# mmbajo/PROBA-V

Measured on AMD Instinct MI355X. Metric: LR-patches/sec fwd+bwd (WDSR-B r12 t9, 16x16, bs128), higher is better.
Workload: dtype f32 (products as 3 scaled-fp16-piece MFMA products, f32 accumulate)

## Files before the change

### proba-v_amd/csrc/kernels_cw4.hip

```cpp
#include "kernels_x6.h"
#include "x6_device.h"
#include <cstdlib>
#include <algorithm>

namespace probav {
#ifdef CW4_DIAG
namespace diag {
#endif

struct Cw4Args {
    ConvGeom g;
    int Wp, Wt, nsplit, SR, nstrips, nslot;
    unsigned mTo, mNvr, mTi, mNslot;
};

namespace {
__device__ __forceinline__ int qdiv(int v, int d, unsigned m) { return (int)__umulhi((unsigned)v, m) + (d == 1 ? v : 0); }
unsigned qmagic(int d) { return d <= 1 ? 0u : (unsigned)((0x100000000ull + (unsigned)d - 1) / (unsigned)d); }
typedef float f32x4u __attribute__((ext_vector_type(4), aligned(4)));
typedef unsigned u32x4b __attribute__((ext_vector_type(4)));
constexpr int CW4_PSE = 151;
constexpr int CW4_PS = 16 * CW4_PSE;
constexpr int CW4_ROW = 8 * CW4_PS;
constexpr unsigned CW4_OOB = 0x40000000u;
}

#ifdef CW4_STAMP
__device__ unsigned long long g_cw4_stamps[1024 * 8];
#endif

#define CW4_SBAR() __builtin_amdgcn_sched_barrier(0)
#ifdef CW4_STAMP
#define CW4_ST(k) do { unsigned long long t_; asm volatile("s_memtime %0\n\ts_waitcnt lgkmcnt(0)" : "=s"(t_) :: "memory"); st_acc[k] += t_ - st_prev; st_prev = t_; } while (0)
#ifdef CW4_STAMP_ROUNDS
#define CW4_STR(k) CW4_ST(k)
#else
#define CW4_STR(k) do { } while (0)
#endif
#else
#define CW4_STR(k) do { } while (0)
#define CW4_ST(k) do { } while (0)
#endif

template <int CIN, int COUT, int TP, bool RELU, bool SKIP, bool BIAS>
__global__ __launch_bounds__(256, 1) void conv3_w4_kernel(Cw4Args a, const float* __restrict__ x, const uint4* __restrict__ wfrag, const float* __restrict__ bias,
                                                         const float* __restrict__ skip, float* __restrict__ y, Amax am)
{
    extern __shared__ __attribute__((aligned(16))) unsigned char lds[];
    constexpr int NST = CIN == 25 ? 5 : 6, KB = 9 * NST, G = 3 * KB;
    constexpr int NW1R = CIN == 25 ? 12 : 8;
    constexpr int NCH = CIN == 25 ? 3 : 4;
    constexpr int PS = CW4_PS, ROW = CW4_ROW;
    constexpr int PD = 2;
    constexpr int TO = TP - 2;
    const ConvGeom& g = a.g;
    const int tid = threadIdx.x, lane = tid & 63, half = lane >> 5, col = lane & 31;
    const int wave = __builtin_amdgcn_readfirstlane(tid >> 6);
    const int per = a.nstrips * a.nsplit;
    const int n = blockIdx.x / per, srem = blockIdx.x - n * per;
    const int strip = srem / a.nsplit, sp = srem - strip * a.nsplit;
    const int ws0 = sp * a.Wt, hb = strip * a.SR;
    const int SRr = g.Ho - hb < a.SR ? g.Ho - hb : a.SR;
    const int nvr = a.Wt * g.To, NV = SRr * nvr, NTL = (NV + 31) >> 5, nround = (NTL + 3) >> 2;
    const int NS = a.nslot;
    float omax = 0.f;
#ifdef CW4_STAMP
    unsigned long long st_t0 = __builtin_amdgcn_s_memtime(), st_r0 = __builtin_amdgcn_s_memrealtime();
    unsigned long long st_prev = st_t0, st_acc[8] = {0, 0, 0, 0, 0, 0, 0, 0};
#endif

    const int lw0 = a.nsplit == 1 ? g.pw : 0, Wl = a.nsplit == 1 ? g.Wi : a.Wt + 2;
    const int nvs = Wl * g.Ti, items = nvs * NCH;
    const int ea = h3_exp(am.x[n]);
    const float sa = pow2i(ea);
    int s_srcb[2], s_offb[2];
    float s_sc[2];
    int s3_o[3], s3_offb = 0;
    float s3_sc[3] = {0.f, 0.f, 0.f};
    {
        auto locate = [&](int lv, int& lw, int& t, int& iwc, int& colok) {
            const int lwr = qdiv(lv, g.Ti, a.mTi);
            t = lv - lwr * g.Ti; lw = lw0 + lwr;
            const int iw = ws0 + lw - g.pw;
            colok = (iw >= 0 ? 1 : 0) & (iw < g.Wi ? 1 : 0);
            iwc = iw < 0 ? 0 : (iw < g.Wi ? iw : g.Wi - 1);
        };
#pragma unroll
        for (int k = 0; k < 2; ++k) {
            const int it = tid + 256 * k;
            const int ic = it < items ? it : items - 1;
            const int lv = CIN == 25 ? (int)(((unsigned)ic * 43691u) >> 17) : ic >> 2;
            const int cc = ic - lv * NCH;
            int lw, t, iwc, colok;
            locate(lv, lw, t, iwc, colok);
            s_srcb[k] = ((iwc * g.Ti + t) * CIN + 8 * cc) * 4;
            s_offb[k] = (lw * TO + t) * 16 + cc * PS;
            s_sc[k] = colok ? sa : 0.f;
        }
        if constexpr (CIN == 25) {
            const int lv = tid < nvs ? tid : nvs - 1;
            int lw, t, iwc, colok;
            locate(lv, lw, t, iwc, colok);
            const int base = ((iwc * g.Ti + t) * CIN + 24) * 4;
            s3_offb = (lw * TO + t) * 16 + 3 * PS;
            const int ok3[3] = {colok && t - 1 >= 0, colok, colok && t + 1 < g.Ti};
#pragma unroll
            for (int j = 0; j < 3; ++j) { s3_o[j] = base + (ok3[j] ? (j - 1) * CIN * 4 : 0); s3_sc[j] = ok3[j] ? sa : 0.f; }
        }
    }
    const long xsample = (long)g.Hi * g.Wi * g.Ti * CIN;
    const __amdgpu_buffer_rsrc_t xrs = __builtin_amdgcn_make_buffer_rsrc(const_cast<float*>(x + (long)n * xsample), 0, (unsigned)xsample * 4u, 0x00020000);
    const int xrowb = g.Wi * g.Ti * CIN * 4;
    struct Staged { u32x4b v[2][2]; unsigned g3[3]; };
    auto row_of = [&](int q, int& rowoff, float& rokf) {
        const int ih = hb - g.ph + q;
        const bool rok = ih >= 0 && ih < g.Hi;
        rowoff = (rok ? ih : 0) * xrowb;
        rokf = rok ? 1.f : 0.f;
    };
    auto stage_load_items = [&](int rowoff, Staged& sv) {
#pragma unroll
        for (int k = 0; k < 2; ++k) {
            sv.v[k][0] = __builtin_amdgcn_raw_buffer_load_b128(xrs, s_srcb[k], rowoff, 0);
            sv.v[k][1] = __builtin_amdgcn_raw_buffer_load_b128(xrs, s_srcb[k] + 16, rowoff, 0);
        }
    };
    auto stage_load_g3 = [&](int rowoff, Staged& sv) {
#ifdef CW4_ABL_NOG3
        sv.g3[0] = sv.g3[1] = sv.g3[2] = 0u; return;
#endif
        if constexpr (CIN == 25) {
#pragma unroll
            for (int j = 0; j < 3; ++j) sv.g3[j] = __builtin_amdgcn_raw_buffer_load_b32(xrs, s3_o[j], rowoff, 0);
        }
    };
    auto slot_of = [&](int q) -> int { return (q - qdiv(q, NS, a.mNslot) * NS) * ROW; };
    struct Cut { float sc[2], sg[3]; f32x2 t[4]; unsigned h0[4], h1[4]; float u[3]; };
    constexpr int ROW_MOPS = CIN == 25 ? 52 : 41;
    auto stage_mop = [&](int m, int slot, float rokf, Staged& sv, Cut& c, bool reload, int rel) {
        if (m < 5) {
            if (m < 2) c.sc[m] = s_sc[m] * rokf;
            else if (CIN == 25) c.sg[m - 2] = s3_sc[m - 2] * rokf;
            return;
        }
        m -= 5;
        if (m < 36) {
            const int k = m / 18, i = m % 18;
            if (i < 16) {
                const int p = i >> 2, op = i & 3;
                if (op == 0) {
                    const u32x4b q = sv.v[k][p >> 1];
                    const f32x2 v = {__uint_as_float(q[2 * (p & 1)]), __uint_as_float(q[2 * (p & 1) + 1])};
                    c.t[p] = v * (f32x2){c.sc[k], c.sc[k]};
                    if (p == 3 && reload) {
                        sv.v[k][0] = __builtin_amdgcn_raw_buffer_load_b128(xrs, s_srcb[k], rel, 0);
                        sv.v[k][1] = __builtin_amdgcn_raw_buffer_load_b128(xrs, s_srcb[k] + 16, rel, 0);
                    }
                } else if (op == 1) {
                    c.h0[p] = __builtin_bit_cast(unsigned, __builtin_convertvector(c.t[p], f16x2));
                } else if (op == 2) {
                    asm("v_fma_mixlo_f16 %0, %1, -1.0, %2 op_sel:[0,0,0] op_sel_hi:[1,0,0]" : "=v"(c.h1[p]) : "v"(c.h0[p]), "v"(c.t[p][0]));
                } else {
                    asm("v_fma_mixhi_f16 %0, %1, -1.0, %2 op_sel:[1,0,0] op_sel_hi:[1,0,0]" : "+v"(c.h1[p]) : "v"(c.h0[p]), "v"(c.t[p][1]));
                }
            } else {
#ifdef CW4_ABL_NOWRITE
                asm volatile("" :: "v"(c.h0[0]), "v"(c.h0[1]), "v"(c.h0[2]), "v"(c.h0[3]), "v"(c.h1[0]), "v"(c.h1[1]), "v"(c.h1[2]), "v"(c.h1[3]));
                return;
#endif
                unsigned char* ent = lds + slot + s_offb[k];
                if (i == 16) *reinterpret_cast<uint4*>(ent) = make_uint4(c.h0[0], c.h0[1], c.h0[2], c.h0[3]);
                else *reinterpret_cast<uint4*>(ent + 4 * PS) = make_uint4(c.h1[0], c.h1[1], c.h1[2], c.h1[3]);
            }
            return;
        }
        if constexpr (CIN == 25) {
            m -= 36;
            if (m < 3) { c.u[m] = __uint_as_float(sv.g3[m]) * c.sg[m]; if (m == 2 && reload) stage_load_g3(rel, sv); }
            else if (m == 3) c.h0[0] = __builtin_bit_cast(unsigned, __builtin_convertvector((f32x2){c.u[0], c.u[1]}, f16x2));
            else if (m == 4) c.h0[1] = __builtin_bit_cast(unsigned, __builtin_convertvector((f32x2){c.u[2], 0.f}, f16x2));
            else if (m == 5) asm("v_fma_mixlo_f16 %0, %1, -1.0, %2 op_sel:[0,0,0] op_sel_hi:[1,0,0]" : "=v"(c.h1[0]) : "v"(c.h0[0]), "v"(c.u[0]));
            else if (m == 6) asm("v_fma_mixhi_f16 %0, %1, -1.0, %2 op_sel:[1,0,0] op_sel_hi:[1,0,0]" : "+v"(c.h1[0]) : "v"(c.h0[0]), "v"(c.u[1]));
            else if (m == 7) c.h1[1] = 0u;
            else if (m == 8) asm("v_fma_mixlo_f16 %0, %1, -1.0, %2 op_sel:[0,0,0] op_sel_hi:[1,0,0]" : "+v"(c.h1[1]) : "v"(c.h0[1]), "v"(c.u[2]));
            else if (m == 9) *reinterpret_cast<uint2*>(lds + slot + s3_offb) = make_uint2(c.h0[0], c.h0[1]);
            else *reinterpret_cast<uint2*>(lds + slot + s3_offb + 4 * PS) = make_uint2(c.h1[0], c.h1[1]);
        }
    };
    auto need = [&](int r) -> int {
        const int vlast = (r + 1) * 128 - 1 < NV - 1 ? (r + 1) * 128 - 1 : NV - 1;
        return qdiv(vlast, nvr, a.mNvr) + 2;
    };

    CW4_ST(3);
    int hiq = nround > 0 ? need(0) : -1;
    Staged p0[4];
    int p0_slot[4];
    float p0_rok[4];
#pragma unroll
    for (int q = 0; q < 4; ++q) {
        int rowoff;
        row_of(q <= hiq ? q : 0, rowoff, p0_rok[q]);
        p0_slot[q] = slot_of(q <= hiq ? q : 0);
        stage_load_items(rowoff, p0[q]);
        stage_load_g3(rowoff, p0[q]);
    }
    constexpr int NQ = ((KB - NW1R) * 64 + 255) / 256;
    u32x4b w1q[NQ];
    const u32x4b* wfrag4 = reinterpret_cast<const u32x4b*>(wfrag);
    const int Z0c = a.Wp * (TP - 2);
    constexpr int NF = KB + NW1R, NF4 = (NF + 3) / 4;
    u32x4b xq[NF4];
#pragma unroll
    for (int i = 0; i < NF4; ++i) {
        int f = 4 * i + wave;
        f = f < NF ? f : NF - 1;
        xq[i] = wfrag4[(f < KB ? 2 * f : 2 * (f - KB) + 1) * 64 + lane];
    }
    const int tab = NS * ROW + (KB - NW1R) * 1024;
    const int tc = tid < g.Cout ? tid : 0;
    const unsigned tew = am.w[tc];
    const float tbv = (bias ? bias : reinterpret_cast<const float*>(am.w))[tc];
#pragma unroll
    for (int i = 0; i < NQ; ++i) {
        int e = tid + 256 * i;
        e = e < (KB - NW1R) * 64 ? e : (KB - NW1R) * 64 - 1;
        w1q[i] = wfrag4[(2 * (NW1R + (e >> 6)) + 1) * 64 + (e & 63)];
    }
    CW4_ST(4);
    if (tid < 32) {
        const int e = -(ea + h3_exp_w(tew));
        reinterpret_cast<int*>(lds + tab)[tid] = e;
        reinterpret_cast<float*>(lds + tab + 128)[tid] = (BIAS && bias && tid < g.Cout) ? ldexpf(tbv, -e) : 0.f;
    }
#pragma unroll
    for (int i = 0; i < NF4; ++i) {
        int f = 4 * i + wave;
        f = f < NF ? f : NF - 1;
        *reinterpret_cast<u32x4b*>(lds + f * 1024 + lane * 16) = xq[i];
    }
    asm volatile("s_waitcnt lgkmcnt(0)\n\ts_barrier" ::: "memory");
    f16x8 w0[KB], w1r[NW1R > 0 ? NW1R : 1];
#pragma unroll
    for (int K = 0; K < KB; ++K) { Frag f; f.u = *reinterpret_cast<const uint4*>(lds + K * 1024 + lane * 16); w0[K] = f.h; }
#pragma unroll
    for (int K = 0; K < NW1R; ++K) { Frag f; f.u = *reinterpret_cast<const uint4*>(lds + (KB + K) * 1024 + lane * 16); w1r[K] = f.h; }
#pragma unroll
    for (int K = 0; K < KB; ++K) asm volatile("" : "+a"(w0[K]));
#pragma unroll
    for (int K = 0; K < NW1R; ++K) asm volatile("" : "+a"(w1r[K]));
    asm volatile("s_waitcnt lgkmcnt(0)\n\ts_barrier" ::: "memory");
    if (a.nsplit == 1) {
        uint4* z = reinterpret_cast<uint4*>(lds);
        for (int i = tid; i < NS * ROW / 16; i += 256) z[i] = make_uint4(0u, 0u, 0u, 0u);
    } else {
        const int nzone = CW4_PSE - Z0c, nplanes = NS * 8;
        for (int i = tid; i < nzone * nplanes; i += 256) {
            const int pl = i / nzone, e = i - pl * nzone;
            *reinterpret_cast<uint4*>(lds + pl * PS + (Z0c + e) * 16) = make_uint4(0u, 0u, 0u, 0u);
        }
        if constexpr (CIN == 25) {
            for (int i = tid; i < Z0c * NS * 2; i += 256) {
                const int pl = i / Z0c, e = i - pl * Z0c;
                *reinterpret_cast<uint4*>(lds + (pl >> 1) * ROW + (3 + 4 * (pl & 1)) * PS + e * 16) = make_uint4(0u, 0u, 0u, 0u);
            }
        }
    }
    asm volatile("s_waitcnt lgkmcnt(0)\n\ts_barrier" ::: "memory");
    CW4_ST(5);
#pragma unroll
    for (int q = 0; q < 4; ++q) {
        Cut c;
#pragma unroll
        for (int m = 0; m < ROW_MOPS; ++m) stage_mop(m, p0_slot[q], p0_rok[q], p0[q], c, false, 0);
    }
    CW4_ST(6);
    const int w1a = NS * ROW + lane * 16;
#pragma unroll
    for (int i = 0; i < NQ; ++i) {
        int e = tid + 256 * i;
        e = e < (KB - NW1R) * 64 ? e : (KB - NW1R) * 64 - 1;
        *reinterpret_cast<u32x4b*>(lds + NS * ROW + e * 16) = w1q[i];
    }
    int eun[16];
    f32x16 bias16;
#pragma unroll
    for (int jj = 0; jj < 4; ++jj) {
        const int4 e4 = *reinterpret_cast<const int4*>(lds + tab + (8 * jj + 4 * half) * 4);
        const float4 b4 = *reinterpret_cast<const float4*>(lds + tab + 128 + (8 * jj + 4 * half) * 4);
        eun[4 * jj] = e4.x; eun[4 * jj + 1] = e4.y; eun[4 * jj + 2] = e4.z; eun[4 * jj + 3] = e4.w;
        bias16[4 * jj] = b4.x; bias16[4 * jj + 1] = b4.y; bias16[4 * jj + 2] = b4.z; bias16[4 * jj + 3] = b4.w;
    }
    const float lo = g.relu ? 0.f : -__builtin_inff();
    (void)lo;
    if (BIAS) asm volatile("" : "+a"(bias16));
    CW4_ST(7);
    asm volatile("s_waitcnt lgkmcnt(0)\n\ts_barrier" ::: "memory");

    const long out_base = ((long)n * g.Ho + hb) * g.Wo * g.To;
    const unsigned ybytes = (unsigned)(SRr * g.Wo * g.To * g.Cout) * 4u;
    const __amdgpu_buffer_rsrc_t yrs = __builtin_amdgcn_make_buffer_rsrc(y + out_base * g.Cout, 0, ybytes, 0x00020000);
    const __amdgpu_buffer_rsrc_t srs = __builtin_amdgcn_make_buffer_rsrc(const_cast<float*>(skip ? skip + out_base * g.Cout : y), 0, skip ? ybytes : 0u, 0x00020000);
    unsigned cofs[4];
#pragma unroll
    for (int jj = 0; jj < 4; ++jj) cofs[jj] = 8 * jj + 4 * half < COUT ? 4u * (8 * jj + 4 * half) : CW4_OOB;

    int offH[5];
    {
        const int pA[5] = {0, 2, 1, 0, 2}, pB[5] = {1, 0, 2, 1, 3};
#pragma unroll
        for (int st = 0; st < 5; ++st) offH[st] = (half ? pB[st] : pA[st]) * PS;
    }
    const int Z0 = a.Wp * TO;
    struct TileTmp { int vi, hrel, rem, w, t, x, e0, s0, s1, s2, b0, b1, b2, dlo, dhi; unsigned yo; };
    constexpr int TILE_STEPS = 14;
    auto tile_step = [&](int step, int tile, TileTmp& q, int (&bs)[9], unsigned (&eo)[4]) {
#define CW4_PIN(v) asm volatile("" : "+v"(v))
        if (step == 0) { const int v = tile * 32 + col; q.vi = v < NV ? v : NV - 1; q.yo = v < NV ? 0u : CW4_OOB; CW4_PIN(q.vi); CW4_PIN(q.yo); }
        if (step == 1) { q.hrel = (int)__umulhi((unsigned)q.vi, a.mNvr); q.rem = q.vi - q.hrel * nvr; CW4_PIN(q.hrel); CW4_PIN(q.rem); }
        if (step == 2) { q.w = (int)__umulhi((unsigned)q.rem, a.mTo); q.t = q.rem - q.w * g.To; CW4_PIN(q.w); CW4_PIN(q.t); }
        if (step == 3) { q.x = q.w * TO + q.t; q.s0 = q.hrel - (int)__umulhi((unsigned)q.hrel, a.mNslot) * NS; CW4_PIN(q.x); CW4_PIN(q.s0); }
        if (step == 4) { q.s1 = q.s0 + 1 < NS ? q.s0 + 1 : q.s0 + 1 - NS; q.e0 = q.x * 16 + (CIN == 32 ? half * PS : 0); CW4_PIN(q.s1); CW4_PIN(q.e0); }
        if (step == 5) { q.s2 = q.s1 + 1 < NS ? q.s1 + 1 : q.s1 + 1 - NS; CW4_PIN(q.s2); }
        if (step == 6) { q.b0 = q.s0 * ROW + q.e0; q.b1 = q.s1 * ROW + q.e0; q.b2 = q.s2 * ROW + q.e0; bs[1] = q.b0; bs[4] = q.b1; bs[7] = q.b2; CW4_PIN(bs[1]); CW4_PIN(bs[4]); CW4_PIN(bs[7]); }
        if (step == 7) { const int z = ((q.x - 1 - Z0) & 15) + Z0 - q.x; q.dlo = q.t == 0 ? z * 16 : -16; CW4_PIN(q.dlo); }
        if (step == 8) { const int z = ((q.x + 1 - Z0) & 15) + Z0 - q.x; q.dhi = q.t == TO - 1 ? z * 16 : 16; CW4_PIN(q.dhi); }
        if (step == 9) { bs[0] = q.b0 + q.dlo; bs[3] = q.b1 + q.dlo; bs[6] = q.b2 + q.dlo; CW4_PIN(bs[0]); CW4_PIN(bs[3]); CW4_PIN(bs[6]); }
        if (step == 10) { bs[2] = q.b0 + q.dhi; bs[5] = q.b1 + q.dhi; bs[8] = q.b2 + q.dhi; CW4_PIN(bs[2]); CW4_PIN(bs[5]); CW4_PIN(bs[8]); }
        if (step == 11) { q.yo += (unsigned)(((q.hrel * g.Wo + ws0 + q.w) * g.To + q.t) * COUT) * 4u; CW4_PIN(q.yo); }
        if (step == 12) { eo[0] = q.yo + cofs[0]; eo[1] = q.yo + cofs[1]; CW4_PIN(eo[0]); CW4_PIN(eo[1]); }
        if (step == 13) { eo[2] = q.yo + cofs[2]; eo[3] = q.yo + cofs[3]; CW4_PIN(eo[2]); CW4_PIN(eo[3]); }
#undef CW4_PIN
    };
    int adr5[5] = {0, 0, 0, 0, 0};
    auto read_A = [&](const int (&bs)[9], int K, Frag (&af)[2]) {
        const int gg = K / NST, st = K % NST, dh = gg / 3, dw = gg % 3;
        if constexpr (CIN == 25) {
            if (dw == 0) {
                const int bm = bs[3 * dh], bz = bs[3 * dh + 1], bp = bs[3 * dh + 2];
                const int b = st == 0 ? bm : st == 1 ? (half ? bz : bm) : st == 2 ? bz : st == 3 ? bp : (half ? bz : bp);
                adr5[st] = b + offH[st];
            }
            const unsigned char* p = lds + adr5[st];
            af[0].u = *reinterpret_cast<const uint4*>(p + dw * TO * 16);
            af[1].u = *reinterpret_cast<const uint4*>(p + dw * TO * 16 + 4 * PS);
        } else {
            const int d = st >> 1, kb = st & 1;
            const unsigned char* p = lds + bs[3 * dh + d];
            af[0].u = *reinterpret_cast<const uint4*>(p + dw * TO * 16 + 2 * kb * PS);
            af[1].u = *reinterpret_cast<const uint4*>(p + dw * TO * 16 + 2 * kb * PS + 4 * PS);
        }
    };
    auto read_W1 = [&](int K, Frag& wf) {
        if (K >= NW1R) wf.u = *reinterpret_cast<const uint4*>(lds + w1a + (K - NW1R) * 1024);
    };

    CW4_ST(2);
    f32x16 accA, accB;
#pragma unroll
    for (int i = 0; i < 16; ++i) { accA[i] = 0.f; accB[i] = 0.f; }
#ifdef CW4_ABL_2ACC
    f32x16 acc2;
    for (int i = 0; i < 16; ++i) acc2[i] = 0.f;
#endif
    f32x4u skq[4];
#pragma unroll
    for (int jj = 0; jj < 4; ++jj) skq[jj] = (f32x4u){0.f, 0.f, 0.f, 0.f};
    int bs[9];
    unsigned eo[4], eo_prev[4] = {CW4_OOB, CW4_OOB, CW4_OOB, CW4_OOB};
    {
        TileTmp q;
#pragma unroll
        for (int st = 0; st < TILE_STEPS; ++st) tile_step(st, wave, q, bs, eo);
    }
    Frag A[PD + 1][2], W1[PD + 1];
#pragma unroll
    for (int K = 0; K < PD; ++K) { read_A(bs, K, A[K]); read_W1(K, W1[K]); }

    Staged sv[2];
    auto round = [&](int r, f32x16& acc, f32x16& pacc) __attribute__((always_inline)) {
        const int hi_next = r + 1 < nround ? need(r + 1) : hiq;
        const int hi_nn = r + 2 < nround ? need(r + 2) : hi_next;
        const int q0 = hiq + 1, q1 = hi_next - hiq >= 2 ? hiq + 2 : hiq + 1;
        const int n0 = hi_next + 1, n1 = hi_nn - hi_next >= 2 ? hi_next + 2 : hi_next + 1;
        int rowoff[2], slot[2];
        float rokf[2], rokn;
        int dummy;
        row_of(q0, dummy, rokf[0]); row_of(q1, dummy, rokf[1]);
        row_of(n0, rowoff[0], rokn); row_of(n1, rowoff[1], rokn);
        slot[0] = slot_of(q0); slot[1] = slot_of(q1);
        Cut cut;
        TileTmp tq;
        int nbs[9];
        unsigned neo[4];
        float m2 = 0.f;
#pragma unroll
        for (int K = 0; K < KB; ++K) {
#pragma unroll
            for (int j = 0; j < 3; ++j) {
                const int gp = 3 * K + j;
                const int sl = K % (PD + 1);
                {
                    f16x8 wa;
                    if (j == 1) { if (K < NW1R) wa = w1r[K < NW1R ? K : 0]; else wa = W1[sl].h; }
                    else wa = w0[K];
                    const f16x8 xb = (j == 0) ? A[sl][1].h : A[sl][0].h;
                    if (gp == 0) {
                        if (BIAS) acc = __builtin_amdgcn_mfma_f32_32x32x16_f16(wa, xb, bias16, 0, 0, 0);
                        else {
                            f32x16 zero;
#pragma unroll
                            for (int i = 0; i < 16; ++i) zero[i] = 0.f;
                            acc = __builtin_amdgcn_mfma_f32_32x32x16_f16(wa, xb, zero, 0, 0, 0);
                        }
                    } else acc = __builtin_amdgcn_mfma_f32_32x32x16_f16(wa, xb, acc, 0, 0, 0);
                }
                CW4_SBAR();
#ifndef CW4_ABL_NOREAD
                if (j == 0) {
                    const int KN = K + PD, sn = KN % (PD + 1);
#ifndef CW4_ABL_W1LATE
                    read_W1(KN < KB ? KN : KN - KB, W1[sn]);
#endif
                    if (KN < KB) read_A(bs, KN, A[sn]); else read_A(nbs, KN - KB, A[sn]);
                }
#ifdef CW4_ABL_W1LATE
                if (j == 1) {
                    const int KN = K + PD, sn = KN % (PD + 1);
                    read_W1(KN < KB ? KN : KN - KB, W1[sn]);
                }
#endif
#endif
                if (K >= 1 && K <= 10 && j == 1) tile_step(K - 1, 4 * (r + 1) + wave, tq, nbs, neo);
                if (K >= 12 && K <= 15 && j == 1) tile_step(K - 2, 4 * (r + 1) + wave, tq, nbs, neo);
                if (K == 11 && j == 1) { CW4_STR(3); asm volatile("s_barrier" ::: "memory"); CW4_STR(4); }
#ifndef CW4_ABL_NOEPI
                if (K < 16 && j == 2) {
                    const int e = K, jj = e >> 2, i = e & 3;
                    float v = ldexpf(pacc[e], eun[e]);
                    if (RELU) v = fmaxf(v, lo);
                    const float o = SKIP ? v + skq[jj][i] : v;
                    skq[jj][i] = o;
                    if ((e & 1) == 0) m2 = o; else asm volatile("v_max3_f32 %0, %0, |%1|, |%2|" : "+v"(omax) : "v"(m2), "v"(o));
                }
                if (j == 1 && (K == 4 || K == 8 || K == 12 || K == 16)) {
                    const int jj = K / 4 - 1;
                    const u32x4b o = {__float_as_uint(skq[jj][0]), __float_as_uint(skq[jj][1]), __float_as_uint(skq[jj][2]), __float_as_uint(skq[jj][3])};
                    if (COUT == 32 || jj < 3) __builtin_amdgcn_raw_buffer_store_b128(o, yrs, eo_prev[jj], 0, 0);
                    else __builtin_amdgcn_raw_buffer_store_b32(o[0], yrs, eo_prev[jj], 0, 0);
                    if (K == 16) omax = r == 0 ? 0.f : omax;
                }
                if (SKIP && (K == 17 || K == 18) && j > 0) {
                    const int jj = 2 * (K - 17) + j - 1;
                    if (COUT == 32 || jj < 3) {
                        const u32x4b q = __builtin_amdgcn_raw_buffer_load_b128(srs, eo[jj], 0, 0);
                        skq[jj] = (f32x4u){__uint_as_float(q[0]), __uint_as_float(q[1]), __uint_as_float(q[2]), __uint_as_float(q[3])};
                    } else {
                        const unsigned q = __builtin_amdgcn_raw_buffer_load_b32(srs, eo[jj], 0, 0);
                        skq[jj] = (f32x4u){__uint_as_float(q), 0.f, 0.f, 0.f};
                    }
                }
#endif
#ifndef CW4_ABL_NOSTAGE
                {
                    constexpr int NKS = (2 * ROW_MOPS + 5) / 6, KS0 = KB - PD - NKS;
                    if (K >= KS0 && K < KS0 + NKS && j > 0) {
                        const int m0 = (K - KS0) * 6 + 3 * (j - 1);
#pragma unroll
                        for (int m = m0; m < m0 + 3; ++m)
                            if (m < 2 * ROW_MOPS) {
#ifdef CW4_ABL_NOCUT
                                if (m == 0) asm volatile("" :: "v"(sv[0].v[0][0]), "v"(sv[0].v[1][1]), "v"(sv[1].v[0][0]), "v"(sv[1].v[1][1]));
                                continue;
#endif
                                stage_mop(m % ROW_MOPS, slot[m / ROW_MOPS], rokf[m / ROW_MOPS], sv[m / ROW_MOPS], cut, true, rowoff[m / ROW_MOPS]);
                            }
                    }
                }
#endif
                CW4_SBAR();
            }
        }
        CW4_STR(5);
#pragma unroll
        for (int d = 0; d < 9; ++d) bs[d] = nbs[d];
#pragma unroll
        for (int jj = 0; jj < 4; ++jj) { eo_prev[jj] = eo[jj]; eo[jj] = neo[jj]; }
        hiq = hi_next;
    };
    {
        const int hi1 = 1 < nround ? need(1) : hiq;
        const int n0 = hiq + 1, n1 = hi1 - hiq >= 2 ? hiq + 2 : hiq + 1;
        int ro;
        float rk;
        row_of(n0, ro, rk); stage_load_items(ro, sv[0]); stage_load_g3(ro, sv[0]);
        row_of(n1, ro, rk); stage_load_items(ro, sv[1]); stage_load_g3(ro, sv[1]);
    }
#pragma unroll 1
    for (int r = 0; r < nround; r += 2) {
        round(r, accA, accB);
        round(r + 1, accB, accA);
    }
    {
#pragma unroll
        for (int e = 0; e < 16; ++e) {
            const int jj = e >> 2, i = e & 3;
            float v = ldexpf(accB[e], eun[e]);
            if (RELU) v = fmaxf(v, lo);
            const float o = SKIP ? v + skq[jj][i] : v;
            skq[jj][i] = o;
            omax = fmaxf(omax, fabsf(o));
        }
        if (nround == 0) omax = 0.f;
#pragma unroll
        for (int jj = 0; jj < 4; ++jj) {
            const u32x4b o = {__float_as_uint(skq[jj][0]), __float_as_uint(skq[jj][1]), __float_as_uint(skq[jj][2]), __float_as_uint(skq[jj][3])};
            if (COUT == 32 || jj < 3) __builtin_amdgcn_raw_buffer_store_b128(o, yrs, eo_prev[jj], 0, 0);
            else __builtin_amdgcn_raw_buffer_store_b32(o[0], yrs, eo_prev[jj], 0, 0);
        }
    }
#ifdef CW4_ABL_2ACC
    for (int i = 0; i < 16; ++i) omax += acc2[i];
#endif
    if (am.y) amax_commit(omax, am.y + n);
#ifdef CW4_STAMP
    if (lane == 0 && blockIdx.x < 256) {
        unsigned long long* o = g_cw4_stamps + (blockIdx.x * 4 + wave) * 8;
        o[0] = __builtin_amdgcn_s_memtime() - st_t0; o[1] = __builtin_amdgcn_s_memrealtime() - st_r0;
        for (int k = 2; k < 8; ++k) o[k] = st_acc[k];
    }
#endif
}

static bool cw4_plan(const ConvGeom& g, Cw4Args& p, size_t& lds_bytes, int& grid)
{
    if (g.kh != 3 || g.kw != 3 || g.kt != 3 || g.reflect_hw || g.reflect_t) return false;
    if (!((g.Cin == 25 && g.Cout == 32) || (g.Cin == 32 && (g.Cout == 25 || g.Cout == 32)))) return false;
    if (g.ph != 1 || g.pw != 1 || g.pt != 1) return false;
    if (g.Ho != g.Hi || g.Wo != g.Wi || g.To != g.Ti) return false;
    if (g.To != 9 && g.To != 7) return false;
    if (g.Ho < 3) return false;
    const int Tp = g.To + 2;
    for (int ns = 1; ns <= 4; ++ns) {
        if (g.Wo % ns) continue;
        const int wt = g.Wo / ns, nvr = wt * g.To;
        const int wp = wt + 2;
        const int nvs = (ns == 1 ? g.Wi : wt + 2) * g.Ti, items = nvs * (g.Cin == 25 ? 3 : 4);
        if (items > 512 || nvs > 256 || nvr < 64 || wp * g.To + 16 + 2 * g.To > CW4_PSE) continue;
        int nstrips = (256 + g.N * ns - 1) / (g.N * ns);
        if (nstrips < 1) nstrips = 1;
        if (nstrips > g.Ho / 4) nstrips = g.Ho / 4 > 0 ? g.Ho / 4 : 1;
        const int SR = (g.Ho + nstrips - 1) / nstrips;
        nstrips = (g.Ho + SR - 1) / SR;
        const int NV = SR * nvr, nround = ((NV + 31) / 32 + 3) / 4;
        auto needf = [&](int r) { const int vl = std::min(NV - 1, (r + 1) * 128 - 1); return vl / nvr + 2; };
        int nslot = needf(0) + 1;
        for (int r = 0; r + 1 < nround; ++r) nslot = std::max(nslot, needf(r + 1) - (r * 128) / nvr + 1);
        const int kb = g.Cin == 25 ? 45 : 54, nw1r = g.Cin == 25 ? 12 : 8;
        const size_t need = (size_t)nslot * CW4_ROW + (size_t)(kb - nw1r) * 1024 + 256;
        if (need > 163840) continue;
        p.g = g; p.Wp = wp; p.Wt = wt; p.nsplit = ns; p.SR = SR; p.nstrips = nstrips; p.nslot = nslot;
        p.mTo = qmagic(g.To); p.mNvr = qmagic(nvr); p.mTi = qmagic(g.Ti); p.mNslot = qmagic(nslot);
        lds_bytes = need; grid = g.N * nstrips * ns;
        return true;
    }
    return false;
}

bool cw4_conv_supported(const ConvGeom& g, const float* gate)
{
    Cw4Args p;
    size_t lds_bytes;
    int grid;
    return gate == nullptr && cw4_plan(g, p, lds_bytes, grid);
}

int cw4_conv_forward(const ConvGeom& g, const float* x, const float* wfrag, const float* bias, const float* skip, float* y, const Amax& am, hipStream_t s)
{
    Cw4Args p;
    size_t lds_bytes;
    int grid;
    if (!cw4_plan(g, p, lds_bytes, grid)) { set_error("cw4_conv_forward: unsupported geometry", hipSuccess); return PROBAV_EINVAL; }
    if (!am.x || !am.w) { set_error("cw4_conv_forward: H3 arithmetic needs the operands' amax slots", hipSuccess); return PROBAV_EINVAL; }
#define CW4_LAUNCH(C, O, T, R, S, B) return launch_lds<conv3_w4_kernel<C, O, T, R, S, B>>("conv3_w4", dim3(grid), dim3(256), lds_bytes, s, p, x, (const uint4*)wfrag, bias, skip, y, am)
#define CW4_LAUNCH_T(C, O) do { if (g.To == 9) CW4_LAUNCH(C, O, 11, true, true, true); else CW4_LAUNCH(C, O, 9, true, true, true); } while (0)
    if (g.Cin == 25 && g.To == 9 && !g.relu && skip && bias) CW4_LAUNCH(25, 32, 11, false, true, true);
    else if (g.Cin == 32 && g.Cout == 25 && g.To == 9 && !g.relu && !skip && !bias) CW4_LAUNCH(32, 25, 11, false, false, false);
    else if (g.Cin == 25) CW4_LAUNCH_T(25, 32);
    else if (g.Cout == 25) CW4_LAUNCH_T(32, 25);
    else CW4_LAUNCH_T(32, 32);
#undef CW4_LAUNCH_T
#undef CW4_LAUNCH
}

#ifdef CW4_DIAG
}
#endif
}
```

Before: 21990.

## Use 16x16x32 f16 MFMA path for Cin=32 conv3 with new staging layout

Adds a separate main loop for 32-input-channel layers that issues mfma_f32_16x16x32_f16 on 16-voxel tiles instead of the previous MFMA form. To feed that instruction shape, it re-lays out the LDS staging (plane stride 152, a different item-to-channel mapping, and weight fragment offsets), moves the scale and bias tables, and rebuilds the tile address computation, epilogue and store scheduling. The goal is fewer instruction issues and better MFMA throughput per K step. The cost is a large amount of new code and a change to the LDS budget, so there is a real risk of layout or bank conflicts and correctness bugs in the new path.

```diff
diff --git a/proba-v_amd/csrc/kernels_cw4.hip b/proba-v_amd/csrc/kernels_cw4.hip
--- a/proba-v_amd/csrc/kernels_cw4.hip
+++ b/proba-v_amd/csrc/kernels_cw4.hip
@@ -2,10 +2,16 @@
 #include "x6_device.h"
 #include <cstdlib>
 #include <algorithm>
+#include <type_traits>
 
 namespace probav {
 #ifdef CW4_DIAG
 namespace diag {
+#endif
+#ifdef CW4_ABL_K16
+#define CW4_K32_FORM false
+#else
+#define CW4_K32_FORM true
 #endif
 
 struct Cw4Args {
@@ -19,9 +25,10 @@
 unsigned qmagic(int d) { return d <= 1 ? 0u : (unsigned)((0x100000000ull + (unsigned)d - 1) / (unsigned)d); }
 typedef float f32x4u __attribute__((ext_vector_type(4), aligned(4)));
 typedef unsigned u32x4b __attribute__((ext_vector_type(4)));
-constexpr int CW4_PSE = 151;
-constexpr int CW4_PS = 16 * CW4_PSE;
-constexpr int CW4_ROW = 8 * CW4_PS;
+typedef float f32x4a __attribute__((ext_vector_type(4)));
+constexpr bool cw4_k32(int cin) { return cin == 32 && CW4_K32_FORM; }
+constexpr int cw4_pse(int cin) { return cw4_k32(cin) ? 152 : 151; }
+constexpr int cw4_row(int cin) { return 8 * 16 * cw4_pse(cin); }
 constexpr unsigned CW4_OOB = 0x40000000u;
 }
 
@@ -50,7 +57,8 @@
     constexpr int NST = CIN == 25 ? 5 : 6, KB = 9 * NST, G = 3 * KB;
     constexpr int NW1R = CIN == 25 ? 12 : 8;
     constexpr int NCH = CIN == 25 ? 3 : 4;
-    constexpr int PS = CW4_PS, ROW = CW4_ROW;
+    constexpr bool K32 = cw4_k32(CIN);
+    constexpr int PSE = cw4_pse(CIN), PS = 16 * PSE, ROW = 8 * PS;
     constexpr int PD = 2;
     constexpr int TO = TP - 2;
     const ConvGeom& g = a.g;
@@ -89,8 +97,13 @@
         for (int k = 0; k < 2; ++k) {
             const int it = tid + 256 * k;
             const int ic = it < items ? it : items - 1;
-            const int lv = CIN == 25 ? (int)(((unsigned)ic * 43691u) >> 17) : ic >> 2;
-            const int cc = ic - lv * NCH;
+            int lv = CIN == 25 ? (int)(((unsigned)ic * 43691u) >> 17) : ic >> 2;
+            int cc = ic - lv * NCH;
+            if constexpr (K32) {
+                const int i16 = it & 15;
+                if ((it >> 6) < (nvs >> 4)) { lv = 4 * (it >> 4) + ((i16 >> 1) & 3); cc = (i16 & 1) + 2 * (i16 >> 3); }
+                else { lv = 16 * (it >> 6) + i16; lv = lv < nvs ? lv : nvs - 1; cc = (it >> 4) & 3; }
+            }
             int lw, t, iwc, colok;
             locate(lv, lw, t, iwc, colok);
             s_srcb[k] = ((iwc * g.Ti + t) * CIN + 8 * cc) * 4;
@@ -217,7 +230,7 @@
         f = f < NF ? f : NF - 1;
         xq[i] = wfrag4[(f < KB ? 2 * f : 2 * (f - KB) + 1) * 64 + lane];
     }
-    const int tab = NS * ROW + (KB - NW1R) * 1024;
+    const int tab = K32 ? NF * 1024 : NS * ROW + (KB - NW1R) * 1024;
     const int tc = tid < g.Cout ? tid : 0;
     const unsigned tew = am.w[tc];
     const float tbv = (bias ? bias : reinterpret_cast<const float*>(am.w))[tc];
@@ -241,10 +254,23 @@
     }
     asm volatile("s_waitcnt lgkmcnt(0)\n\ts_barrier" ::: "memory");
     f16x8 w0[KB], w1r[NW1R > 0 ? NW1R : 1];
-#pragma unroll
-    for (int K = 0; K < KB; ++K) { Frag f; f.u = *reinterpret_cast<const uint4*>(lds + K * 1024 + lane * 16); w0[K] = f.h; }
-#pragma unroll
-    for (int K = 0; K < NW1R; ++K) { Frag f; f.u = *reinterpret_cast<const uint4*>(lds + (KB + K) * 1024 + lane * 16); w1r[K] = f.h; }
+    const int ck = 2 * ((lane >> 4) & 1) + (lane >> 5);
+    const int fro = K32 ? (ck >> 1) * 1024 + ((lane & 15) + 32 * (ck & 1)) * 16 : lane * 16;
+#pragma unroll
+    for (int K = 0; K < KB; ++K) { Frag f; f.u = *reinterpret_cast<const uint4*>(lds + (K32 ? (K >> 1) * 2048 + (K & 1) * 256 : K * 1024) + fro); w0[K] = f.h; }
+#pragma unroll
+    for (int K = 0; K < NW1R; ++K) { Frag f; f.u = *reinterpret_cast<const uint4*>(lds + KB * 1024 + (K32 ? (K >> 1) * 2048 + (K & 1) * 256 : K * 1024) + fro); w1r[K] = f.h; }
+    int eun32[8];
+    f32x4a bias32[2];
+    if constexpr (K32) {
+#pragma unroll
+        for (int v = 0; v < 2; ++v) {
+            const int4 e4 = *reinterpret_cast<const int4*>(lds + tab + (16 * v + 4 * (lane >> 4)) * 4);
+            const float4 b4 = *reinterpret_cast<const float4*>(lds + tab + 128 + (16 * v + 4 * (lane >> 4)) * 4);
+            eun32[4 * v] = e4.x; eun32[4 * v + 1] = e4.y; eun32[4 * v + 2] = e4.z; eun32[4 * v + 3] = e4.w;
+            bias32[v] = (f32x4a){b4.x, b4.y, b4.z, b4.w};
+        }
+    }
 #pragma unroll
     for (int K = 0; K < KB; ++K) asm volatile("" : "+a"(w0[K]));
 #pragma unroll
@@ -254,7 +280,7 @@
         uint4* z = reinterpret_cast<uint4*>(lds);
         for (int i = tid; i < NS * ROW / 16; i += 256) z[i] = make_uint4(0u, 0u, 0u, 0u);
     } else {
-        const int nzone = CW4_PSE - Z0c, nplanes = NS * 8;
+        const int nzone = PSE - Z0c, nplanes = NS * 8;
         for (int i = tid; i < nzone * nplanes; i += 256) {
             const int pl = i / nzone, e = i - pl * nzone;
             *reinterpret_cast<uint4*>(lds + pl * PS + (Z0c + e) * 16) = make_uint4(0u, 0u, 0u, 0u);
@@ -275,7 +301,7 @@
         for (int m = 0; m < ROW_MOPS; ++m) stage_mop(m, p0_slot[q], p0_rok[q], p0[q], c, false, 0);
     }
     CW4_ST(6);
-    const int w1a = NS * ROW + lane * 16;
+    const int w1a = NS * ROW + fro;
 #pragma unroll
     for (int i = 0; i < NQ; ++i) {
         int e = tid + 256 * i;
@@ -285,7 +311,7 @@
     int eun[16];
     f32x16 bias16;
 #pragma unroll
-    for (int jj = 0; jj < 4; ++jj) {
+    for (int jj = 0; jj < (K32 ? 0 : 4); ++jj) {
         const int4 e4 = *reinterpret_cast<const int4*>(lds + tab + (8 * jj + 4 * half) * 4);
         const float4 b4 = *reinterpret_cast<const float4*>(lds + tab + 128 + (8 * jj + 4 * half) * 4);
         eun[4 * jj] = e4.x; eun[4 * jj + 1] = e4.y; eun[4 * jj + 2] = e4.z; eun[4 * jj + 3] = e4.w;
@@ -293,7 +319,8 @@
     }
     const float lo = g.relu ? 0.f : -__builtin_inff();
     (void)lo;
-    if (BIAS) asm volatile("" : "+a"(bias16));
+    if (BIAS && !K32) asm volatile("" : "+a"(bias16));
+    if (BIAS && K32) { asm volatile("" : "+a"(bias32[0])); asm volatile("" : "+a"(bias32[1])); }
     CW4_ST(7);
     asm volatile("s_waitcnt lgkmcnt(0)\n\ts_barrier" ::: "memory");
 
@@ -312,6 +339,208 @@
         for (int st = 0; st < 5; ++st) offH[st] = (half ? pB[st] : pA[st]) * PS;
     }
     const int Z0 = a.Wp * TO;
+
+    auto finish = [&]() {
+        if (am.y) amax_commit(omax, am.y + n);
+#ifdef CW4_STAMP
+        if (lane == 0 && blockIdx.x < 256) {
+            unsigned long long* o = g_cw4_stamps + (blockIdx.x * 4 + wave) * 8;
+            o[0] = __builtin_amdgcn_s_memtime() - st_t0; o[1] = __builtin_amdgcn_s_memrealtime() - st_r0;
+            for (int k = 2; k < 8; ++k) o[k] = st_acc[k];
+        }
+#endif
+    };
+    if constexpr (K32) {
+        constexpr int NT = 27, NEO = COUT == 32 ? 2 : 3;
+        const int n16 = lane & 15, kq = lane >> 4;
+        unsigned cof[NEO];
+        cof[0] = 16u * kq;
+        cof[1] = (COUT == 32 || kq < 2) ? 64u + 16u * kq : CW4_OOB;
+        if constexpr (COUT == 25) cof[2] = kq == 2 ? 96u : CW4_OOB;
+        struct Tile32 { int v, vi, hrel, rem, w, t, x, e0, s0, s1, s2, b0, b1, b2, zl, zh, dlo, dhi; unsigned yo; };
+        constexpr int TILE_PIECES = 21;
+        auto tstep = [&](int pc, int u, int tile, Tile32& q, int (&b)[9], unsigned (&o)[NEO]) {
+#define CW4_PIN(v) asm volatile("" : "+v"(v))
+            if (pc == 0) { q.v = tile * 32 + 16 * u + n16; q.vi = q.v < NV ? q.v : NV - 1; CW4_PIN(q.v); CW4_PIN(q.vi); }
+            if (pc == 1) { q.yo = q.v < NV ? 0u : CW4_OOB; CW4_PIN(q.yo); }
+            if (pc == 2) { q.hrel = (int)__umulhi((unsigned)q.vi, a.mNvr); q.rem = q.vi - q.hrel * nvr; CW4_PIN(q.hrel); CW4_PIN(q.rem); }
+            if (pc == 3) { q.w = (int)__umulhi((unsigned)q.rem, a.mTo); q.t = q.rem - q.w * g.To; CW4_PIN(q.w); CW4_PIN(q.t); }
+            if (pc == 4) { q.x = q.w * TO + q.t; CW4_PIN(q.x); }
+            if (pc == 5) { q.s0 = q.hrel - (int)__umulhi((unsigned)q.hrel, a.mNslot) * NS; CW4_PIN(q.s0); }
+            if (pc == 6) { q.s1 = q.s0 + 1 < NS ? q.s0 + 1 : q.s0 + 1 - NS; CW4_PIN(q.s1); }
+            if (pc == 7) { q.e0 = q.x * 16 + ck * PS; CW4_PIN(q.e0); }
+            if (pc == 8) { q.s2 = q.s1 + 1 < NS ? q.s1 + 1 : q.s1 + 1 - NS; CW4_PIN(q.s2); }
+            if (pc == 9) { q.b0 = q.s0 * ROW + q.e0; q.b1 = q.s1 * ROW + q.e0; b[1] = q.b0; b[4] = q.b1; CW4_PIN(b[1]); CW4_PIN(b[4]); }
+            if (pc == 10) { q.b2 = q.s2 * ROW + q.e0; b[7] = q.b2; CW4_PIN(b[7]); }
+            if (pc == 11) { q.zl = (((q.x - 1 - Z0) & 15) + Z0 - q.x) * 16; CW4_PIN(q.zl); }
+            if (pc == 12) { q.dlo = q.t == 0 ? q.zl : -16; CW4_PIN(q.dlo); }
+            if (pc == 13) { q.zh = (((q.x + 1 - Z0) & 15) + Z0 - q.x) * 16; CW4_PIN(q.zh); }
+            if (pc == 14) { q.dhi = q.t == TO - 1 ? q.zh : 16; CW4_PIN(q.dhi); }
+            if (pc == 15) { b[0] = q.b0 + q.dlo; b[3] = q.b1 + q.dlo; b[6] = q.b2 + q.dlo; CW4_PIN(b[0]); CW4_PIN(b[3]); CW4_PIN(b[6]); }
+            if (pc == 16) { b[2] = q.b0 + q.dhi; b[5] = q.b1 + q.dhi; b[8] = q.b2 + q.dhi; CW4_PIN(b[2]); CW4_PIN(b[5]); CW4_PIN(b[8]); }
+            if (pc == 17) { q.rem = (q.hrel * g.Wo + ws0 + q.w) * g.To + q.t; CW4_PIN(q.rem); }
+            if (pc == 18) { q.yo += (unsigned)(q.rem * COUT) * 4u; CW4_PIN(q.yo); }
+            if (pc == 19) { o[0] = q.yo + cof[0]; o[1] = q.yo + cof[1]; CW4_PIN(o[0]); CW4_PIN(o[1]); }
+            if (pc == 20) { if constexpr (COUT == 25) { o[2] = q.yo + cof[2]; CW4_PIN(o[2]); } }
+#undef CW4_PIN
+        };
+        auto read_X = [&](const int (&b)[9], int T, int pc, Frag& xf) {
+            const int gg = T / 3, d = T % 3, dh = gg / 3, dw = gg % 3;
+            xf.u = *reinterpret_cast<const uint4*>(lds + b[3 * dh + d] + dw * TO * 16 + pc * 4 * PS);
+        };
+        auto read_W = [&](int T, int v, Frag& wf) {
+            if (2 * T >= NW1R) wf.u = *reinterpret_cast<const uint4*>(lds + w1a + (2 * T - NW1R) * 1024 + v * 256);
+        };
+        auto store_y = [&](int u, int v, const f32x4u& val, const unsigned (&o)[NEO]) {
+            (void)u;
+            const u32x4b q = {__float_as_uint(val[0]), __float_as_uint(val[1]), __float_as_uint(val[2]), __float_as_uint(val[3])};
+            __builtin_amdgcn_raw_buffer_store_b128(q, yrs, o[v], 0, 0);
+            if constexpr (COUT == 25) { if (v == 1) __builtin_amdgcn_raw_buffer_store_b32(q[0], yrs, o[2], 0, 0); }
+        };
+        f32x4a accA[4], accB[4];
+#pragma unroll
+        for (int i = 0; i < 4; ++i) { accA[i] = (f32x4a){0.f, 0.f, 0.f, 0.f}; accB[i] = (f32x4a){0.f, 0.f, 0.f, 0.f}; }
+        f32x4u skq[4];
+#pragma unroll
+        for (int i = 0; i < 4; ++i) skq[i] = (f32x4u){0.f, 0.f, 0.f, 0.f};
+        int bs[2][9];
+        unsigned eo[2][NEO], eo_prev[2][NEO];
+#pragma unroll
+        for (int u = 0; u < 2; ++u)
+#pragma unroll
+            for (int i = 0; i < NEO; ++i) eo_prev[u][i] = CW4_OOB;
+        {
+            Tile32 q[2];
+#pragma unroll
+            for (int pc = 0; pc < TILE_PIECES; ++pc) { tstep(pc, 0, wave, q[0], bs[0], eo[0]); tstep(pc, 1, wave, q[1], bs[1], eo[1]); }
+        }
+        Frag X[2][2][2], W1[2][2];
+        read_X(bs[0], 0, 1, X[0][0][1]); read_X(bs[1], 0, 1, X[0][1][1]); read_W(0, 0, W1[0][0]);
+        read_X(bs[0], 0, 0, X[0][0][0]); read_W(0, 1, W1[0][1]); read_X(bs[1], 0, 0, X[0][1][0]);
+        Staged sv[2];
+        auto round = [&](int r, auto par, f32x4a (&acc)[4], f32x4a (&pacc)[4]) __attribute__((always_inline)) {
+            constexpr int PAR = decltype(par)::value;
+            const int hi_next = r + 1 < nround ? need(r + 1) : hiq;
+            const int hi_nn = r + 2 < nround ? need(r + 2) : hi_next;
+            const int q0 = hiq + 1, q1 = hi_next - hiq >= 2 ? hiq + 2 : hiq + 1;
+            const int n0 = hi_next + 1, n1 = hi_nn - hi_next >= 2 ? hi_next + 2 : hi_next + 1;
+            int rowoff[2], slot[2];
+            float rokf[2], rokn;
+            int dummy;
+            row_of(q0, dummy, rokf[0]); row_of(q1, dummy, rokf[1]);
+            row_of(n0, rowoff[0], rokn); row_of(n1, rowoff[1], rokn);
+            slot[0] = slot_of(q0); slot[1] = slot_of(q1);
+            Cut cut;
+            Tile32 tq[2];
+            int nbs[2][9];
+            unsigned neo[2][NEO];
+            float m2 = 0.f;
+#pragma unroll
+            for (int T = 0; T < NT; ++T) {
+#pragma unroll
+                for (int j = 0; j < 12; ++j) {
+                    const int pr = j >> 2, u = (j >> 1) & 1, v = j & 1, sl = (T + PAR) & 1, sn = sl ^ 1;
+                    {
+                        f16x8 wa;
+                        if (pr == 1) { if (2 * T < NW1R) wa = w1r[2 * T < NW1R ? 2 * T + v : 0]; else wa = W1[sl][v].h; }
+                        else wa = w0[2 * T + v];
+                        const f16x8 xb = pr == 0 ? X[sl][u][1].h : X[sl][u][0].h;
+                        if (T == 0 && pr == 0) acc[2 * u + v] = __builtin_amdgcn_mfma_f32_16x16x32_f16(wa, xb, BIAS ? bias32[v] : (f32x4a){0.f, 0.f, 0.f, 0.f}, 0, 0, 0);
+                        else acc[2 * u + v] = __builtin_amdgcn_mfma_f32_16x16x32_f16(wa, xb, acc[2 * u + v], 0, 0, 0);
+                    }
+                    CW4_SBAR();
+#ifndef CW4_ABL_NOREAD
+                    if (j < 6) {
+                        const int TN = T + 1 < NT ? T + 1 : 0;
+                        auto request = [&](const int (&nb)[2][9]) {
+                            if (j == 0) read_X(nb[1], TN, 1, X[sn][1][1]);
+                            if (j == 1) read_X(nb[0], TN, 1, X[sn][0][1]);
+                            if (j == 2) read_W(TN, 1, W1[sn][1]);
+                            if (j == 3) read_X(nb[1], TN, 0, X[sn][1][0]);
+                            if (j == 4) read_W(TN, 0, W1[sn][0]);
+                            if (j == 5) read_X(nb[0], TN, 0, X[sn][0][0]);
+                        };
+                        if (T + 1 < NT) request(bs); else request(nbs);
+                    }
+#endif
+                    if (T == 5 && j == 5) { CW4_STR(3); asm volatile("s_barrier" ::: "memory"); CW4_STR(4); }
+                    if (j >= 6) {
+                        constexpr int S_EPI = 2 * TILE_PIECES, S_SKIP = S_EPI + 20, S_STAGE = S_SKIP + 4;
+                        static_assert(S_STAGE + 2 * ROW_MOPS <= 6 * (NT - 1), "the fillers do not fit the tile");
+                        const int sg = 6 * T + j - 6;
+                        if (sg < S_EPI) tstep(sg >> 1, sg & 1, 4 * (r + 1) + wave, tq[sg & 1], nbs[sg & 1], neo[sg & 1]);
+#ifndef CW4_ABL_NOEPI
+                        if (sg >= S_EPI && sg < S_SKIP) {
+                            const int uv = (sg - S_EPI) / 5, i = (sg - S_EPI) % 5;
+                            if (i < 4) {
+                                float val = ldexpf(pacc[uv][i], eun32[4 * (uv & 1) + i]);
+                                if (RELU) val = fmaxf(val, lo);
+                                const float o = SKIP ? val + skq[uv][i] : val;
+                                skq[uv][i] = o;
+                                if ((i & 1) == 0) m2 = o; else asm volatile("v_max3_f32 %0, %0, |%1|, |%2|" : "+v"(omax) : "v"(m2), "v"(o));
+                            } else {
+                                store_y(uv >> 1, uv & 1, skq[uv], eo_prev[uv >> 1]);
+                                if (uv == 3) omax = r == 0 ? 0.f : omax;
+                            }
+                        }
+                        if (SKIP && sg >= S_SKIP && sg < S_STAGE) {
+                            const int uv = sg - S_SKIP, su = uv >> 1, sv_ = uv & 1;
+                            u32x4b q = __builtin_amdgcn_raw_buffer_load_b128(srs, eo[su][sv_], 0, 0);
+                            if constexpr (COUT == 25) { if (sv_ == 1) q[0] |= __builtin_amdgcn_raw_buffer_load_b32(srs, eo[su][2], 0, 0); }
+                            skq[uv] = (f32x4u){__uint_as_float(q[0]), __uint_as_float(q[1]), __uint_as_float(q[2]), __uint_as_float(q[3])};
+                        }
+#endif
+#ifndef CW4_ABL_NOSTAGE
+                        if (sg >= S_STAGE && sg < S_STAGE + 2 * ROW_MOPS) {
+                            const int m = sg - S_STAGE;
+                            stage_mop(m % ROW_MOPS, slot[m / ROW_MOPS], rokf[m / ROW_MOPS], sv[m / ROW_MOPS], cut, true, rowoff[m / ROW_MOPS]);
+                        }
+#endif
+                    }
+                    CW4_SBAR();
+                }
+            }
+            CW4_STR(5);
+#pragma unroll
+            for (int u = 0; u < 2; ++u) {
+#pragma unroll
+                for (int d = 0; d < 9; ++d) bs[u][d] = nbs[u][d];
+#pragma unroll
+                for (int i = 0; i < NEO; ++i) { eo_prev[u][i] = eo[u][i]; eo[u][i] = neo[u][i]; }
+            }
+            hiq = hi_next;
+        };
+        {
+            const int hi1 = 1 < nround ? need(1) : hiq;
+            const int n0 = hiq + 1, n1 = hi1 - hiq >= 2 ? hiq + 2 : hiq + 1;
+            int ro;
+            float rk;
+            row_of(n0, ro, rk); stage_load_items(ro, sv[0]);
+            row_of(n1, ro, rk); stage_load_items(ro, sv[1]);
+        }
+        CW4_ST(2);
+#pragma unroll 1
+        for (int r = 0; r < nround; r += 2) {
+            round(r, std::integral_constant<int, 0>{}, accA, accB);
+            round(r + 1, std::integral_constant<int, 1>{}, accB, accA);
+        }
+#pragma unroll
+        for (int uv = 0; uv < 4; ++uv) {
+#pragma unroll
+            for (int i = 0; i < 4; ++i) {
+                float val = ldexpf(accB[uv][i], eun32[4 * (uv & 1) + i]);
+                if (RELU) val = fmaxf(val, lo);
+                const float o = SKIP ? val + skq[uv][i] : val;
+                skq[uv][i] = o;
+                omax = fmaxf(omax, fabsf(o));
+            }
+        }
+        if (nround == 0) omax = 0.f;
+#pragma unroll
+        for (int uv = 0; uv < 4; ++uv) store_y(uv >> 1, uv & 1, skq[uv], eo_prev[uv >> 1]);
+        finish();
+        return;
+    }
     struct TileTmp { int vi, hrel, rem, w, t, x, e0, s0, s1, s2, b0, b1, b2, dlo, dhi; unsigned yo; };
     constexpr int TILE_STEPS = 14;
     auto tile_step = [&](int step, int tile, TileTmp& q, int (&bs)[9], unsigned (&eo)[4]) {
@@ -522,14 +751,7 @@
 #ifdef CW4_ABL_2ACC
     for (int i = 0; i < 16; ++i) omax += acc2[i];
 #endif
-    if (am.y) amax_commit(omax, am.y + n);
-#ifdef CW4_STAMP
-    if (lane == 0 && blockIdx.x < 256) {
-        unsigned long long* o = g_cw4_stamps + (blockIdx.x * 4 + wave) * 8;
-        o[0] = __builtin_amdgcn_s_memtime() - st_t0; o[1] = __builtin_amdgcn_s_memrealtime() - st_r0;
-        for (int k = 2; k < 8; ++k) o[k] = st_acc[k];
-    }
-#endif
+    finish();
 }
 
 static bool cw4_plan(const ConvGeom& g, Cw4Args& p, size_t& lds_bytes, int& grid)
@@ -546,7 +768,7 @@
         const int wt = g.Wo / ns, nvr = wt * g.To;
         const int wp = wt + 2;
         const int nvs = (ns == 1 ? g.Wi : wt + 2) * g.Ti, items = nvs * (g.Cin == 25 ? 3 : 4);
-        if (items > 512 || nvs > 256 || nvr < 64 || wp * g.To + 16 + 2 * g.To > CW4_PSE) continue;
+        if (items > 512 || nvs > 256 || nvr < 64 || wp * g.To + 16 + 2 * g.To > cw4_pse(g.Cin)) continue;
         int nstrips = (256 + g.N * ns - 1) / (g.N * ns);
         if (nstrips < 1) nstrips = 1;
         if (nstrips > g.Ho / 4) nstrips = g.Ho / 4 > 0 ? g.Ho / 4 : 1;
@@ -557,7 +779,7 @@
         int nslot = needf(0) + 1;
         for (int r = 0; r + 1 < nround; ++r) nslot = std::max(nslot, needf(r + 1) - (r * 128) / nvr + 1);
         const int kb = g.Cin == 25 ? 45 : 54, nw1r = g.Cin == 25 ? 12 : 8;
-        const size_t need = (size_t)nslot * CW4_ROW + (size_t)(kb - nw1r) * 1024 + 256;
+        const size_t need = (size_t)nslot * cw4_row(g.Cin) + (size_t)(kb - nw1r) * 1024 + (cw4_k32(g.Cin) ? 0 : 256);
         if (need > 163840) continue;
         p.g = g; p.Wp = wp; p.Wt = wt; p.nsplit = ns; p.SR = SR; p.nstrips = nstrips; p.nslot = nslot;
         p.mTo = qmagic(g.To); p.mNvr = qmagic(nvr); p.mTi = qmagic(g.Ti); p.mNslot = qmagic(nslot);
```

Result: no change. 22180, median of 6 (+0.8%).
